# rail-berkeley/serl

Hardware: AMD Instinct MI355X
Metric: learner grad-steps/sec (DrQ, bs256, 2x128x128 img) (higher is better)
Workload: dtype f32 (trunk convs as split-fp16 MFMA x3, fp32 accumulate; <=1e-6 vs fp64); 1 GPU; async_drq_sim (DrQ, ResNet-10 frozen trunk, REDQ-10 critic); workload_key=drq, global_batch=256, per_gpu_batch=256, cameras=2, state_dim=24, act_dim=6, replay_capacity=200000, replay_fill=20000, parallelism=dp1, encoder=resnet-pretrained, trunk_passes_per_grad_step=2, trunk_arithmetic=f16x3, schedule=trunk(i+1) overlapped with update(i) on a 2nd stream; gather(i+2) on a 3rd

## Files before the change

serl_amd/csrc/trunk_f16x3_rowslab.h:

```cpp
#pragma once
#include "trunk_f16x3_dma.h"

namespace serl {

__device__ __forceinline__ void rowtile_epilogue(const ConvArgsB& ab, f32x16 (&acc)[2][2], f32x16 (&accx)[2][2], int m0, int n0,
                                                 int n_img, int wave, int li, int lh) {
  const ConvArgs& a = ab.c;
  constexpr int TM = 2, TN = 2, WROWS = 64;
  const int wrow0 = m0 + wave * WROWS;
  float winv[TN];
#pragma unroll
  for (int tn = 0; tn < TN; ++tn) winv[tn] = ab.winv[n0 + tn * 32 + li];
#pragma unroll
  for (int tm = 0; tm < TM; ++tm)
#pragma unroll
    for (int tn = 0; tn < TN; ++tn)
#pragma unroll
      for (int r = 0; r < 16; ++r) acc[tm][tn][r] = (acc[tm][tn][r] + accx[tm][tn][r] * kLoInv) * winv[tn];
#pragma unroll
  for (int tm = 0; tm < TM; ++tm)
#pragma unroll
    for (int r = 0; r < 16; ++r) {
      const int m = wrow0 + tm * 32 + (r & 3) + 8 * (r >> 2) + 4 * lh;
      float* o = a.out + (size_t)m * a.Cout + n0 + li;
#pragma unroll
      for (int tn = 0; tn < TN; ++tn) o[32 * tn] = acc[tm][tn][r];
    }
  const int gsize = a.Cout / kGnGroups;
  double* stp = a.stats + (size_t)n_img * kGnGroups * 2;
#pragma unroll
  for (int tn = 0; tn < TN; ++tn) {
    float s = 0.f, q = 0.f;
#pragma unroll
    for (int tm = 0; tm < TM; ++tm)
#pragma unroll
      for (int r = 0; r < 16; ++r) {
        const float v = acc[tm][tn][r];
        s += v;
        q += v * v;
      }
    stats_flush(s, q, stp, n0 + tn * 32 + li, gsize, true, false);
  }
}

__device__ __forceinline__ void rowtile_epilogue_t(const ConvArgsB& ab, f32x16 (&acc)[2][2], f32x16 (&accx)[2][2], int m0, int n0,
                                                   int n_img, int wave, int lane, int tile_id, uint8_t* lds) {
  const ConvArgs& a = ab.c;
  const FuseArgs& fz = ab.fz;
  constexpr int TM = 2, TN = 2, WROWS = 64;
  const int li = lane & 31, lh = lane >> 5;
  const int wrow0 = m0 + wave * WROWS;
  if (ab.wprio == 2) __builtin_amdgcn_s_setprio(1);
  float winv[TN];
#pragma unroll
  for (int tn = 0; tn < TN; ++tn) winv[tn] = ab.winv[n0 + tn * 32 + li];
#pragma unroll
  for (int tm = 0; tm < TM; ++tm)
#pragma unroll
    for (int tn = 0; tn < TN; ++tn)
#pragma unroll
      for (int r = 0; r < 16; ++r) acc[tm][tn][r] = (acc[tm][tn][r] + accx[tm][tn][r] * kLoInv) * winv[tn];
  const bool local = fz.expected == 0;
  const int gsize = a.Cout / kGnGroups;
  __shared__ float s_part[4][8];
  __shared__ float s_mr[4][2];
#pragma unroll
  for (int tn = 0; tn < TN; ++tn) {
    float s = 0.f, q = 0.f;
#pragma unroll
    for (int tm = 0; tm < TM; ++tm)
#pragma unroll
      for (int r = 0; r < 16; ++r) { const float v = acc[tm][tn][r]; s += v; q += v * v; }
#pragma unroll
    for (int off = 1; off < 16; off <<= 1) { s += __shfl_xor(s, off); q += __shfl_xor(q, off); }
    s += __shfl_xor(s, 32);
    q += __shfl_xor(q, 32);
    if ((lane & 15) == 0 && lane < 32) {
      s_part[wave][(tn * 2 + (lane >> 4)) * 2] = s;
      s_part[wave][(tn * 2 + (lane >> 4)) * 2 + 1] = q;
    }
  }
  __syncthreads();
  if (!local) gnx_publish<0>(fz, tile_id, wave, lane, &s_part[0][0]);
  float* tile = reinterpret_cast<float*>(lds) + wave * (64 * 64);
#pragma unroll
  for (int tm = 0; tm < TM; ++tm)
#pragma unroll
    for (int tn = 0; tn < TN; ++tn)
#pragma unroll
      for (int r = 0; r < 16; ++r) tile[(tm * 32 + (r & 3) + 8 * (r >> 2) + 4 * lh) * 64 + tn * 32 + li] = acc[tm][tn][r];
  const int g8 = lane & 7, rsub = lane >> 3, c0 = n0 + 8 * g8;
  const size_t rowb = (size_t)a.Cout * 4;
  const uint8_t* res_base = fz.mode == 2 ? fz.res_split + (size_t)wrow0 * rowb + c0 * 4
                                         : reinterpret_cast<const uint8_t*>(fz.res_raw) + (size_t)wrow0 * rowb + c0 * 4;
  u32x4 rres[8][2];
  if (fz.mode >= 2) {
#pragma unroll
    for (int p = 0; p < 8; ++p) {
      const uint8_t* q = res_base + (size_t)(8 * p + rsub) * rowb;
      rres[p][0] = *reinterpret_cast<const u32x4*>(q);
      rres[p][1] = *reinterpret_cast<const u32x4*>(q + 16);
    }
  }
  float sc[8], sh[8], rs[8], rh[8];
  {
    float rstd, mf;
    if (local) {
      const int nseg = gsize >> 4, seg0 = (8 * g8 / gsize) * nseg;
      double s0 = 0.0, s1 = 0.0;
      for (int j = 0; j < nseg; ++j) {
        const int k = 2 * (seg0 + j);
        s0 += (((double)s_part[0][k] + (double)s_part[1][k]) + (double)s_part[2][k]) + (double)s_part[3][k];
        s1 += (((double)s_part[0][k + 1] + (double)s_part[1][k + 1]) + (double)s_part[2][k + 1]) + (double)s_part[3][k + 1];
      }
      const double mean = s0 * fz.gn.inv_count, m2 = s1 * fz.gn.inv_count;
      const float var = fmaxf((float)(m2 - mean * mean), 0.f);
      rstd = rsqrtf(var + 1e-5f); mf = (float)mean;
    } else {
      gnx_collect<0>(fz, tile_id, a.tiles_n, n0, wave, lane, &s_part[0][0], s_mr);
      mf = s_mr[g8 >> 1][0]; rstd = s_mr[g8 >> 1][1];
    }
#pragma unroll
    for (int j = 0; j < 8; ++j) { sc[j] = fz.gn.gamma[c0 + j] * rstd; sh[j] = fz.gn.beta[c0 + j] - mf * sc[j]; rs[j] = 0.f; rh[j] = 0.f; }
    if (fz.mode >= 3) {
#pragma unroll
      for (int j = 0; j < 8; ++j) gn_coef1(fz.res_gn, n_img, c0 + j, rs[j], rh[j]);
    }
  }
  uint8_t* out_base = fz.out_split + (size_t)wrow0 * rowb + c0 * 4;
#pragma unroll
  for (int p = 0; p < 8; ++p) {
    const int row = 8 * p + rsub;
    const float4 t0 = *reinterpret_cast<const float4*>(tile + row * 64 + 8 * g8);
    const float4 t1 = *reinterpret_cast<const float4*>(tile + row * 64 + 8 * g8 + 4);
    float v[8] = {t0.x, t0.y, t0.z, t0.w, t1.x, t1.y, t1.z, t1.w};
#pragma unroll
    for (int j = 0; j < 8; ++j) v[j] = v[j] * sc[j] + sh[j];
    if (fz.mode == 2) {
#pragma unroll
      for (int j = 0; j < 4; ++j) {
        const uint32_t wh = rres[p][0][j], wl = rres[p][1][j];
        const h16x2 hh = __builtin_bit_cast(h16x2, wh), ll = __builtin_bit_cast(h16x2, wl);
        v[2 * j] = ((float)hh[0] + (float)ll[0] * kLoInv) + v[2 * j];
        v[2 * j + 1] = ((float)hh[1] + (float)ll[1] * kLoInv) + v[2 * j + 1];
      }
    } else if (fz.mode >= 3) {
#pragma unroll
      for (int j = 0; j < 8; ++j) {
        const uint32_t wx = rres[p][j >> 2][j & 3];
        const float x = __builtin_bit_cast(float, wx);
        const float y = x * rs[j] + rh[j];
        v[j] = (fz.mode == 4 ? fmaxf(y, 0.f) : y) + v[j];
      }
    }
    u32x4 hi, lo;
#pragma unroll
    for (int j = 0; j < 4; ++j) {
      const float a0 = fmaxf(v[2 * j], 0.f), a1 = fmaxf(v[2 * j + 1], 0.f);
      const h16x2 hp = __builtin_amdgcn_cvt_pkrtz(a0, a1);
      const f32x2 rem = {(a0 - (float)hp[0]) * kLoScale, (a1 - (float)hp[1]) * kLoScale};
      const f16x2 lp = __builtin_convertvector(rem, f16x2);
      hi[j] = __builtin_bit_cast(uint32_t, hp);
      lo[j] = __builtin_bit_cast(uint32_t, lp);
    }
    uint8_t* o = out_base + (size_t)row * rowb;
    *reinterpret_cast<u32x4*>(o) = hi;
    *reinterpret_cast<u32x4*>(o + 16) = lo;
  }
}

constexpr int kRowslabPix = 340;
constexpr int kRowslabLds = 2 * 4 * (kRowslabPix * 16 + 32) + 2 * 3 * 2 * 2 * (64 * 16 + 64);
__global__ __launch_bounds__(256, 2) void conv3x3_rowslab_f16x3_kernel(ConvArgsB ab) {
  const ConvArgs& a = ab.c;
  constexpr int TM = 2, TN = 2, WROWS = 64, BM = 256, BN = 64;
  constexpr int A_REGION = kRowslabPix * 16 + 32, A_BYTES = 4 * A_REGION;
  constexpr int B_HALF = BN * 16 + 64, B_PLANE = 2 * B_HALF, B_TAP = 2 * B_PLANE, B_BYTES = 3 * B_TAP;
  static_assert(2 * A_BYTES + 2 * B_BYTES == kRowslabLds, "LDS size of the launch");
  static_assert(3 * 4096 <= B_BYTES, "three DMA pieces per weight buffer");
  constexpr int AJ = 2;
  static_assert(3 * AJ * 256 >= kRowslabPix * 4, "a slab is fetched in three parts");
  extern __shared__ __attribute__((aligned(16))) uint8_t smemb[];
  uint8_t* const smA = smemb;
  uint8_t* const smB = smemb + 2 * A_BYTES;
  const int tid = threadIdx.x, lane = tid & 63, wave = tid >> 6;
  if (ab.wprio) __builtin_amdgcn_s_setprio(3);
  if (ab.stagger > 0 && blockIdx.x >= 256u && blockIdx.x < 512u)
    for (int i = 0; i < ab.stagger; ++i) __builtin_amdgcn_s_sleep(127);
  const int id = (ab.fz.mode && ab.fz.expected) ? fused_tile(ab.fz, gridDim.x) : xcd_remap((int)blockIdx.x, gridDim.x);
  const int bn = id % a.tiles_n, bm = id / a.tiles_n;
  const int m0 = bm * BM, n0 = bn * BN;
  const int n_img = m0 / a.P, oy0 = (m0 - n_img * a.P) / a.Wo;
  const int pw = a.Wo + 2, npix = (BM / a.Wo + 2) * pw;
  const int c16n = a.Cin >> 4, nchunks = 3 * c16n;
  int rbase[3][AJ];
  unsigned okbits = 0;
  __shared__ float s_gn[2][128];
  if (tid < a.Cin) gn_coef1(a.in_gn, n_img, tid, s_gn[0][tid], s_gn[1][tid]);
#pragma unroll
  for (int part = 0; part < 3; ++part) {
    const int v = part * 256 + tid, pix = v >> 1, kh = v & 1;
    const int sy = pix / pw, sx = pix - sy * pw;
    const int iy = oy0 - 1 + sy, ix = sx - 1;
    const int iyc = min(max(iy, 0), a.Hi - 1), ixc = min(max(ix, 0), a.Wi - 1);
    rbase[part][0] = ((n_img * a.Hi + iyc) * a.Wi + ixc) * a.Cin + 8 * kh;
    rbase[part][1] = rbase[part][0] + 4;
    if (pix < npix && iy == iyc && ix == ixc) okbits |= 3u << (part * AJ);
  }
  __syncthreads();
  u32x4 ra[AJ];

#define SERL_RS_LOAD_A(RA, PART, CG)                                                               \
  _Pragma("unroll") for (int j = 0; j < AJ; ++j)                                                   \
    RA[j] = *reinterpret_cast<const u32x4*>(a.in + rbase[PART][j] + ((CG) << 4));
#define SERL_RS_DMA_B(BG, BKY, BBUF)                                                               \
  _Pragma("unroll") for (int kx = 0; kx < 3; ++kx)                                                 \
    __builtin_amdgcn_global_load_lds((gbl_void_t*)(wdsrc + ((size_t)(((BKY) * 3 + kx) * c16n + (BG)) << 12)), \
                                     (lds_void_t*)(smB + (BBUF) * B_BYTES + kx * 4096 + (tid >> 6) * 1024), 16, 0, 0);
#define SERL_RS_STORE_A(RA, PART, ABUF, CGN)                                                       \
  {                                                                                                \
    const int v_ = (PART) * 256 + tid, kh_ = v_ & 1, cb_ = ((CGN) << 4) + 8 * kh_;                 \
    u32x4 hi_ = {0u, 0u, 0u, 0u}, lo_ = {0u, 0u, 0u, 0u};                                          \
    if ((okbits >> ((PART) * AJ)) & 1u) {                                                          \
      _Pragma("unroll") for (int j = 0; j < 2; ++j) {                                              \
        const float4 x_ = __builtin_bit_cast(float4, RA[j]);                                       \
        const float4 sc_ = *reinterpret_cast<const float4*>(&s_gn[0][cb_ + 4 * j]);                \
        const float4 sh_ = *reinterpret_cast<const float4*>(&s_gn[1][cb_ + 4 * j]);                \
        const float4 y_ = make_float4(fmaxf(x_.x * sc_.x + sh_.x, 0.f), fmaxf(x_.y * sc_.y + sh_.y, 0.f), \
                                      fmaxf(x_.z * sc_.z + sh_.z, 0.f), fmaxf(x_.w * sc_.w + sh_.w, 0.f)); \
        uint2 h2_, l2_;                                                                            \
        split4(y_, h2_, l2_);                                                                      \
        hi_[2 * j] = h2_.x; hi_[2 * j + 1] = h2_.y; lo_[2 * j] = l2_.x; lo_[2 * j + 1] = l2_.y;    \
      }                                                                                            \
    }                                                                                              \
    if (v_ < kRowslabPix * 2) {                                                                    \
      uint8_t* d_ = smA + (ABUF) * A_BYTES + (2 * kh_) * A_REGION + (v_ >> 1) * 16;                \
      *reinterpret_cast<u32x4*>(d_) = hi_;                                                         \
      *reinterpret_cast<u32x4*>(d_ + A_REGION) = lo_;                                              \
    }                                                                                              \
  }
#define SERL_RS_LOADS(CG, KY, RA)                                                                  \
  {                                                                                                \
    const int ncg_ = (KY) == 2 ? (CG) + 1 : (CG), nky_ = (KY) == 2 ? 0 : (KY) + 1;                 \
    const int ncgc_ = min(ncg_, c16n - 1), sn_ = min((CG) + 1, c16n - 1);                          \
    SERL_RS_DMA_B(ncgc_, nky_, ((CG) * 3 + (KY) + 1) & 1)                                          \
    if ((KY) == 0) { SERL_RS_LOAD_A(RA, 0, sn_); } else if ((KY) == 1) { SERL_RS_LOAD_A(RA, 1, sn_); } else { SERL_RS_LOAD_A(RA, 2, sn_); } \
  }
#define SERL_RS_STORES(CG, KY, RA)                                                                 \
  {                                                                                                \
    const int sn2_ = min((CG) + 1, c16n - 1);                                                      \
    if ((KY) == 0) { SERL_RS_STORE_A(RA, 0, ((CG) + 1) & 1, sn2_); } else if ((KY) == 1) { SERL_RS_STORE_A(RA, 1, ((CG) + 1) & 1, sn2_); } \
    else { SERL_RS_STORE_A(RA, 2, ((CG) + 1) & 1, sn2_); }                                         \
  }
#define SERL_RS_COMPUTE(C, CG, KY)                                                                 \
  {                                                                                                \
    const uint8_t* sa = smA + ((CG) & 1) * A_BYTES + (KY) * pw * 16;                               \
    const uint8_t* sb = smB + ((C) & 1) * B_BYTES;                                                 \
    _Pragma("unroll") for (int kx = 0; kx < 3; ++kx) {                                             \
      f16x8 ahi[TM], alo[TM], bhi[TN], blo[TN];                                                    \
      _Pragma("unroll") for (int tm = 0; tm < TM; ++tm) {                                          \
        ahi[tm] = *reinterpret_cast<const f16x8*>(sa + arow[tm] + kx * 16);                        \
        alo[tm] = *reinterpret_cast<const f16x8*>(sa + A_REGION + arow[tm] + kx * 16);             \
      }                                                                                            \
      _Pragma("unroll") for (int tn = 0; tn < TN; ++tn) {                                          \
        bhi[tn] = *reinterpret_cast<const f16x8*>(sb + kx * 4096 + wd_bhi[tn]);                    \
        blo[tn] = *reinterpret_cast<const f16x8*>(sb + kx * 4096 + wd_blo[tn]);                    \
      }                                                                                            \
      _Pragma("unroll") for (int tm = 0; tm < TM; ++tm)                                            \
        _Pragma("unroll") for (int tn = 0; tn < TN; ++tn) {                                        \
          accx[tm][tn] = __builtin_amdgcn_mfma_f32_32x32x16_f16(alo[tm], bhi[tn], accx[tm][tn], 0, 0, 0); \
          accx[tm][tn] = __builtin_amdgcn_mfma_f32_32x32x16_f16(ahi[tm], blo[tn], accx[tm][tn], 0, 0, 0); \
          acc[tm][tn] = __builtin_amdgcn_mfma_f32_32x32x16_f16(ahi[tm], bhi[tn], acc[tm][tn], 0, 0, 0); \
        }                                                                                          \
    }                                                                                              \
  }

  f32x16 acc[TM][TN], accx[TM][TN];
#pragma unroll
  for (int tm = 0; tm < TM; ++tm)
#pragma unroll
    for (int tn = 0; tn < TN; ++tn)
#pragma unroll
      for (int r = 0; r < 16; ++r) { acc[tm][tn][r] = 0.f; accx[tm][tn][r] = 0.f; }

  const int li = lane & 31, lh = lane >> 5;
  int arow[TM];
#pragma unroll
  for (int tm = 0; tm < TM; ++tm) {
    const int r = wave * WROWS + tm * 32 + li;
    const int y = r / a.Wo, x = r - y * a.Wo;
    arow[tm] = 2 * lh * A_REGION + (y * pw + x) * 16;
  }
  int wd_bhi[TN], wd_blo[TN];
#pragma unroll
  for (int tn = 0; tn < TN; ++tn) {
    const int row = tn * 32 + li, sw = (row >> 2) & 3;
    wd_bhi[tn] = row * 64 + ((lh ^ sw) << 4);
    wd_blo[tn] = row * 64 + (((2 + lh) ^ sw) << 4);
  }
  const uint8_t* wdsrc = reinterpret_cast<const uint8_t*>(ab.wdma) + (size_t)(n0 >> 6) * (9 * c16n) * 4096 + (tid >> 6) * 1024 + lane * 16;
  SERL_RS_DMA_B(0, 0, 0)
#pragma unroll
  for (int part = 0; part < 3; ++part) {
    SERL_RS_LOAD_A(ra, part, 0);
    SERL_RS_STORE_A(ra, part, 0, 0);
  }
  __syncthreads();
  int cg = 0, ky = 0;
  for (int c = 0; c < nchunks; ++c) {
    SERL_RS_LOADS(cg, ky, ra);
    SERL_RS_COMPUTE(c, cg, ky);
    SERL_RS_STORES(cg, ky, ra);
    __syncthreads();
    if (++ky == 3) { ky = 0; ++cg; }
  }
#undef SERL_RS_LOAD_A
#undef SERL_RS_DMA_B
#undef SERL_RS_STORE_A
#undef SERL_RS_LOADS
#undef SERL_RS_STORES
#undef SERL_RS_COMPUTE
  rowtile_epilogue_t(ab, acc, accx, m0, n0, n_img, wave, lane, id, smemb);
}

constexpr int kSdPieces = 23;
constexpr int kSdSlab = kSdPieces * 1024, kSdW = 3 * 4096;
constexpr int kSlabDmaLds = 2 * kSdSlab + 2 * kSdW;

template <bool EPT = false>
__global__ __launch_bounds__(256, 2) void conv3x3_slabdma_f16x3_kernel(ConvArgsB ab, const uint8_t* zero_page) {
  const ConvArgs& a = ab.c;
  constexpr int TM = 2, TN = 2, WROWS = 64, BM = 256, BN = 64;
  extern __shared__ __attribute__((aligned(16))) uint8_t smemb[];
  uint8_t* const smS = smemb;
  uint8_t* const smW = smemb + 2 * kSdSlab;
  const int tid = threadIdx.x, lane = tid & 63, wave = __builtin_amdgcn_readfirstlane(tid >> 6);
  if (ab.wprio) __builtin_amdgcn_s_setprio(3);
  if (ab.stagger > 0 && blockIdx.x >= 256u && blockIdx.x < 512u)
    for (int i = 0; i < ab.stagger; ++i) __builtin_amdgcn_s_sleep(127);
  const int id = (ab.fz.mode && ab.fz.expected) ? fused_tile(ab.fz, gridDim.x) : xcd_remap((int)blockIdx.x, gridDim.x);
  const int bn = id % a.tiles_n, bm = id / a.tiles_n;
  const int m0 = bm * BM, n0 = bn * BN;
  const int n_img = m0 / a.P, oy0 = (m0 - n_img * a.P) / a.Wo;
  const int pw = a.Wo == 32 ? 34 : 20;
  const int srows = BM / a.Wo + 2;
  const int c16n = a.Cin >> 4, nchunks = 3 * c16n, nslots = 9 * c16n;
  const uint8_t* in_bytes = reinterpret_cast<const uint8_t*>(a.in);
  const uint8_t* zp = zero_page + (lane & 3) * 16;
  unsigned sbase[6], sok = 0;
#pragma unroll
  for (int j = 0; j < 6; ++j) {
    const int pp = 16 * (wave + 4 * j) + (lane >> 2);
    const int sy = pp / pw, sx = pp - sy * pw;
    const int iy = oy0 - 1 + sy, ix = sx - 1;
    const bool ok = sy < srows && sx < a.Wo + 2 && (unsigned)iy < (unsigned)a.Hi && (unsigned)ix < (unsigned)a.Wi;
    const int u = (lane & 3) ^ ((sx >> 2) & 3);
    sbase[j] = ok ? (unsigned)((((long)(n_img * a.Hi + iy) * a.Wi + ix) * a.Cin) * 4 + u * 16) : 0u;
    sok |= (ok ? 1u : 0u) << j;
  }
  const uint8_t* wsrc = reinterpret_cast<const uint8_t*>(ab.wdma) + (size_t)(n0 >> 6) * nslots * 4096 + wave * 1024 + lane * 16;
#define SERL_SD_SLAB(J, CG, SB)                                                                                       \
  if (wave + 4 * (J) < kSdPieces) {                                                                                   \
    const uint8_t* src_ = ((sok >> (J)) & 1u) ? in_bytes + (size_t)sbase[J] + ((CG) << 6) : zp;                       \
    __builtin_amdgcn_global_load_lds((gbl_void_t*)src_, (lds_void_t*)(smS + (SB) * kSdSlab + (wave + 4 * (J)) * 1024), 16, 0, 0); \
  }
#define SERL_SD_W1(CG, KY, WB, KX)                                                                                    \
    __builtin_amdgcn_global_load_lds((gbl_void_t*)(wsrc + ((size_t)(((KY) * 3 + (KX)) * c16n + (CG)) << 12)),        \
                                     (lds_void_t*)(smW + (WB) * kSdW + (KX) * 4096 + wave * 1024), 16, 0, 0);
#define SERL_SD_W(CG, KY, WB) { SERL_SD_W1(CG, KY, WB, 0) SERL_SD_W1(CG, KY, WB, 1) SERL_SD_W1(CG, KY, WB, 2) }
  f32x16 acc[TM][TN], accx[TM][TN];
#pragma unroll
  for (int tm = 0; tm < TM; ++tm)
#pragma unroll
    for (int tn = 0; tn < TN; ++tn)
#pragma unroll
      for (int r = 0; r < 16; ++r) { acc[tm][tn][r] = 0.f; accx[tm][tn][r] = 0.f; }
  const int li = lane & 31, lh = lane >> 5;
  int ahi[TM][3], alo[TM][3];
#pragma unroll
  for (int tm = 0; tm < TM; ++tm) {
    const int r = wave * WROWS + tm * 32 + li;
    const int y = r / a.Wo, x = r - y * a.Wo;
#pragma unroll
    for (int kx = 0; kx < 3; ++kx) {
      const int f = ((x + kx) >> 2) & 3, pa = y * pw + x + kx;
      ahi[tm][kx] = pa * 64 + (((2 * lh) ^ f) << 4);
      alo[tm][kx] = pa * 64 + (((2 * lh + 1) ^ f) << 4);
    }
  }
  int bhi[TN], blo[TN];
#pragma unroll
  for (int tn = 0; tn < TN; ++tn) {
    const int row = tn * 32 + li, sw = (row >> 2) & 3;
    bhi[tn] = row * 64 + ((lh ^ sw) << 4);
    blo[tn] = row * 64 + (((2 + lh) ^ sw) << 4);
  }
#pragma unroll
  for (int j = 0; j < 6; ++j) SERL_SD_SLAB(j, 0, 0)
  SERL_SD_W(0, 0, 0)
  asm volatile("s_waitcnt vmcnt(0)" ::: "memory");
  asm volatile("s_barrier" ::: "memory");
  int cg = 0, ky = 0;
  for (int c = 0; c < nchunks; ++c) {
    const int ncg = ky == 2 ? cg + 1 : cg, nky = ky == 2 ? 0 : ky + 1;
    const int ncgc = min(ncg, c16n - 1), sn = min(cg + 1, c16n - 1);
    SERL_SD_W(ncgc, nky, (c + 1) & 1)
    if (ky == 0) { SERL_SD_SLAB(0, sn, (cg + 1) & 1) SERL_SD_SLAB(1, sn, (cg + 1) & 1) }
    else if (ky == 1) { SERL_SD_SLAB(2, sn, (cg + 1) & 1) SERL_SD_SLAB(3, sn, (cg + 1) & 1) }
    else { SERL_SD_SLAB(4, sn, (cg + 1) & 1) SERL_SD_SLAB(5, sn, (cg + 1) & 1) }
    const uint8_t* sa = smS + (cg & 1) * kSdSlab + ky * pw * 64;
    const uint8_t* sb = smW + (c & 1) * kSdW;
#pragma unroll
    for (int kx = 0; kx < 3; ++kx) {
      f16x8 fah[TM], fal[TM], fbh[TN], fbl[TN];
#pragma unroll
      for (int tm = 0; tm < TM; ++tm) {
        fah[tm] = *reinterpret_cast<const f16x8*>(sa + ahi[tm][kx]);
        fal[tm] = *reinterpret_cast<const f16x8*>(sa + alo[tm][kx]);
      }
#pragma unroll
      for (int tn = 0; tn < TN; ++tn) {
        fbh[tn] = *reinterpret_cast<const f16x8*>(sb + kx * 4096 + bhi[tn]);
        fbl[tn] = *reinterpret_cast<const f16x8*>(sb + kx * 4096 + blo[tn]);
      }
#pragma unroll
      for (int tm = 0; tm < TM; ++tm)
#pragma unroll
        for (int tn = 0; tn < TN; ++tn) {
          accx[tm][tn] = __builtin_amdgcn_mfma_f32_32x32x16_f16(fal[tm], fbh[tn], accx[tm][tn], 0, 0, 0);
          accx[tm][tn] = __builtin_amdgcn_mfma_f32_32x32x16_f16(fah[tm], fbl[tn], accx[tm][tn], 0, 0, 0);
          acc[tm][tn] = __builtin_amdgcn_mfma_f32_32x32x16_f16(fah[tm], fbh[tn], acc[tm][tn], 0, 0, 0);
        }
    }
    asm volatile("s_waitcnt vmcnt(0) lgkmcnt(0)" ::: "memory");
    asm volatile("s_barrier" ::: "memory");
    __builtin_amdgcn_sched_barrier(0);
    if (++ky == 3) { ky = 0; ++cg; }
  }
#undef SERL_SD_SLAB
#undef SERL_SD_W
  if (EPT) rowtile_epilogue_t(ab, acc, accx, m0, n0, n_img, wave, lane, id, smemb);
  else rowtile_epilogue(ab, acc, accx, m0, n0, n_img, wave, li, lh);
}

}
```

Before: 442.6 grad-steps/s.

## Pipeline slab-DMA conv over a six-tap weight ring with counted vmcnt waits

```diff
diff --git a/serl_amd/csrc/trunk_f16x3_rowslab.h b/serl_amd/csrc/trunk_f16x3_rowslab.h
--- a/serl_amd/csrc/trunk_f16x3_rowslab.h
+++ b/serl_amd/csrc/trunk_f16x3_rowslab.h
@@ -324,16 +324,23 @@
 }
 
 constexpr int kSdPieces = 23;
-constexpr int kSdSlab = kSdPieces * 1024, kSdW = 3 * 4096;
-constexpr int kSlabDmaLds = 2 * kSdSlab + 2 * kSdW;
+constexpr int kSdRingTaps = 6, kSdLead = kSdRingTaps - 1;
+constexpr int kSdSlab = kSdPieces * 1024, kSdRing = kSdRingTaps * 4096;
+constexpr int kSlabDmaLds = 2 * kSdSlab + kSdRing;
+constexpr int sd_vmcnt(int kk) {
+  int n = 0;
+  for (int i = 1; i < kSdLead; ++i) n += 1 + ((kk - i + 9) % 9 < 6 ? 1 : 0);
+  return kk == 0 ? n - 1 : n;
+}
+static_assert(sd_vmcnt(0) == 4 && sd_vmcnt(1) == 5 && sd_vmcnt(4) == 8 && sd_vmcnt(8) == 6, "counted waits of the tap ring");
 
 template <bool EPT = false>
-__global__ __launch_bounds__(256, 2) void conv3x3_slabdma_f16x3_kernel(ConvArgsB ab, const uint8_t* zero_page) {
+__global__ __launch_bounds__(256, 2) __attribute__((amdgpu_num_vgpr(108))) void conv3x3_slabdma_f16x3_kernel(ConvArgsB ab, const uint8_t* zero_page) {
   const ConvArgs& a = ab.c;
   constexpr int TM = 2, TN = 2, WROWS = 64, BM = 256, BN = 64;
   extern __shared__ __attribute__((aligned(16))) uint8_t smemb[];
-  uint8_t* const smS = smemb;
-  uint8_t* const smW = smemb + 2 * kSdSlab;
+  uint8_t* const smW = smemb;
+  uint8_t* const smS = smemb + kSdRing;
   const int tid = threadIdx.x, lane = tid & 63, wave = __builtin_amdgcn_readfirstlane(tid >> 6);
   if (ab.wprio) __builtin_amdgcn_s_setprio(3);
   if (ab.stagger > 0 && blockIdx.x >= 256u && blockIdx.x < 512u)
@@ -344,13 +351,14 @@
   const int n_img = m0 / a.P, oy0 = (m0 - n_img * a.P) / a.Wo;
   const int pw = a.Wo == 32 ? 34 : 20;
   const int srows = BM / a.Wo + 2;
-  const int c16n = a.Cin >> 4, nchunks = 3 * c16n, nslots = 9 * c16n;
+  const int c16n = a.Cin >> 4, nslots = 9 * c16n;
   const uint8_t* in_bytes = reinterpret_cast<const uint8_t*>(a.in);
   const uint8_t* zp = zero_page + (lane & 3) * 16;
   unsigned sbase[6], sok = 0;
 #pragma unroll
   for (int j = 0; j < 6; ++j) {
-    const int pp = 16 * (wave + 4 * j) + (lane >> 2);
+    const int pc = wave + 4 * j < kSdPieces ? wave + 4 * j : wave + 4 * j - 4;
+    const int pp = 16 * pc + (lane >> 2);
     const int sy = pp / pw, sx = pp - sy * pw;
     const int iy = oy0 - 1 + sy, ix = sx - 1;
     const bool ok = sy < srows && sx < a.Wo + 2 && (unsigned)iy < (unsigned)a.Hi && (unsigned)ix < (unsigned)a.Wi;
@@ -360,14 +368,16 @@
   }
   const uint8_t* wsrc = reinterpret_cast<const uint8_t*>(ab.wdma) + (size_t)(n0 >> 6) * nslots * 4096 + wave * 1024 + lane * 16;
 #define SERL_SD_SLAB(J, CG, SB)                                                                                       \
-  if (wave + 4 * (J) < kSdPieces) {                                                                                   \
-    const uint8_t* src_ = ((sok >> (J)) & 1u) ? in_bytes + (size_t)sbase[J] + ((CG) << 6) : zp;                       \
-    __builtin_amdgcn_global_load_lds((gbl_void_t*)src_, (lds_void_t*)(smS + (SB) * kSdSlab + (wave + 4 * (J)) * 1024), 16, 0, 0); \
-  }
-#define SERL_SD_W1(CG, KY, WB, KX)                                                                                    \
-    __builtin_amdgcn_global_load_lds((gbl_void_t*)(wsrc + ((size_t)(((KY) * 3 + (KX)) * c16n + (CG)) << 12)),        \
-                                     (lds_void_t*)(smW + (WB) * kSdW + (KX) * 4096 + wave * 1024), 16, 0, 0);
-#define SERL_SD_W(CG, KY, WB) { SERL_SD_W1(CG, KY, WB, 0) SERL_SD_W1(CG, KY, WB, 1) SERL_SD_W1(CG, KY, WB, 2) }
+  {                                                                                                                   \
+    const int pc_ = wave + 4 * (J) < kSdPieces ? wave + 4 * (J) : wave + 4 * (J) - 4;                                 \
+     \
+    unsigned so_ = sbase[J];                                                                                          \
+    asm volatile("" : "+v"(so_));                                                                                     \
+    const uint8_t* src_ = ((sok >> (J)) & 1u) ? in_bytes + (size_t)so_ + ((CG) << 6) : zp;                            \
+    __builtin_amdgcn_global_load_lds((gbl_void_t*)src_, (lds_void_t*)(smS + (SB) * kSdSlab + pc_ * 1024), 16, 0, 0);  \
+  }
+#define SERL_SD_W(SLOT, POS)                                                                                          \
+    __builtin_amdgcn_global_load_lds((gbl_void_t*)(wsrc + ((size_t)(SLOT) << 12)), (lds_void_t*)(smW + (POS) * 4096 + wave * 1024), 16, 0, 0);
   f32x16 acc[TM][TN], accx[TM][TN];
 #pragma unroll
   for (int tm = 0; tm < TM; ++tm)
@@ -376,18 +386,18 @@
 #pragma unroll
       for (int r = 0; r < 16; ++r) { acc[tm][tn][r] = 0.f; accx[tm][tn][r] = 0.f; }
   const int li = lane & 31, lh = lane >> 5;
-  int ahi[TM][3], alo[TM][3];
-#pragma unroll
-  for (int tm = 0; tm < TM; ++tm) {
-    const int r = wave * WROWS + tm * 32 + li;
+  int ahi[3], alo[3];
+  {
+    const int r = wave * WROWS + li;
     const int y = r / a.Wo, x = r - y * a.Wo;
 #pragma unroll
     for (int kx = 0; kx < 3; ++kx) {
       const int f = ((x + kx) >> 2) & 3, pa = y * pw + x + kx;
-      ahi[tm][kx] = pa * 64 + (((2 * lh) ^ f) << 4);
-      alo[tm][kx] = pa * 64 + (((2 * lh + 1) ^ f) << 4);
-    }
-  }
+      ahi[kx] = pa * 64 + (((2 * lh) ^ f) << 4);
+      alo[kx] = pa * 64 + (((2 * lh + 1) ^ f) << 4);
+    }
+  }
+  const int tmo = (32 / a.Wo) * pw * 64;
   int bhi[TN], blo[TN];
 #pragma unroll
   for (int tn = 0; tn < TN; ++tn) {
@@ -395,48 +405,76 @@
     bhi[tn] = row * 64 + ((lh ^ sw) << 4);
     blo[tn] = row * 64 + (((2 + lh) ^ sw) << 4);
   }
+#define SERL_SD_READ_A(SET, KA)                                                                                       \
+  {                                                                                                                   \
+    constexpr int ga_ = (KA) / 9, kya_ = ((KA) % 9) / 3, kxa_ = (KA) % 3;                                             \
+                              \
+    _Pragma("unroll") for (int tm = 0; tm < TM; ++tm) {                                                               \
+      int kyo_ = kya_ * pw * 64 + tm * tmo;                                                                           \
+      asm volatile("" : "+s"(kyo_));                                                                                  \
+      const uint8_t* sa = smS + ga_ * kSdSlab + kyo_;                                                                 \
+      fa[SET][2 * tm] = *reinterpret_cast<const f16x8*>(sa + ahi[kxa_]);                                              \
+      fa[SET][2 * tm + 1] = *reinterpret_cast<const f16x8*>(sa + alo[kxa_]);                                          \
+    }                                                                                                                 \
+  }
+#define SERL_SD_MFMA(TM_, TN_)                                                                                        \
+    accx[TM_][TN_] = __builtin_amdgcn_mfma_f32_32x32x16_f16(fa[cur_][2 * (TM_) + 1], fbh[TN_], accx[TM_][TN_], 0, 0, 0); \
+    acc[TM_][TN_] = __builtin_amdgcn_mfma_f32_32x32x16_f16(fa[cur_][2 * (TM_)], fbh[TN_], acc[TM_][TN_], 0, 0, 0);    \
+    accx[TM_][TN_] = __builtin_amdgcn_mfma_f32_32x32x16_f16(fa[cur_][2 * (TM_)], fbl[TN_], accx[TM_][TN_], 0, 0, 0);
+#define SERL_SD_TAP(K)                                                                                                \
+  {                                                                                                                   \
+    constexpr int g_ = (K) / 9, kk_ = (K) % 9, u_ = (K) + kSdLead, cur_ = (K) & 1;                                    \
+    const uint8_t* sb = smW + ((K) % kSdRingTaps) * 4096;                                                             \
+     \
+    __builtin_amdgcn_sched_barrier(0);                                                                                \
+    asm volatile("s_waitcnt vmcnt(%0) lgkmcnt(0)" ::"n"(sd_vmcnt(kk_)) : "memory");                                   \
+    asm volatile("s_barrier" ::: "memory");                                                                           \
+    __builtin_amdgcn_sched_barrier(0);                                                                                \
+    f16x8 fbh[TN], fbl[TN];                                                                                           \
+    _Pragma("unroll") for (int tn = 0; tn < TN; ++tn) {                                                               \
+      fbh[tn] = *reinterpret_cast<const f16x8*>(sb + bhi[tn]);                                                        \
+      fbl[tn] = *reinterpret_cast<const f16x8*>(sb + blo[tn]);                                                        \
+    }                                                                                                                 \
+    if (kk_ == 0) SERL_SD_READ_A(cur_, K)       \
+                                                \
+    __builtin_amdgcn_sched_barrier(0);                                                                                \
+    if (kk_ < 6) SERL_SD_SLAB((kk_ < 6 ? kk_ : 0), min(cg0 + g_ + 1, c16n - 1), (g_ + 1) & 1)                         \
+    {                                                                                                                 \
+      const int wcg_ = cg0 + u_ / 9;                                                                                  \
+      const int slot_ = wcg_ < c16n ? (u_ % 9) * c16n + wcg_ : nslots - 1;                                            \
+      SERL_SD_W(slot_, u_ % kSdRingTaps)                                                                              \
+    }                                                                                                                 \
+    __builtin_amdgcn_sched_barrier(0);                                                                                \
+    SERL_SD_MFMA(0, 0)                                                                                                \
+     \
+    __builtin_amdgcn_sched_barrier(0);                                                                                \
+    if (kk_ != 8) SERL_SD_READ_A(1 - cur_, (K) + 1)                                                                   \
+    __builtin_amdgcn_sched_barrier(0);                                                                                \
+    SERL_SD_MFMA(0, 1) SERL_SD_MFMA(1, 0) SERL_SD_MFMA(1, 1)                                                          \
+                 \
+    asm volatile("" ::"v"(acc[0][0]), "v"(acc[0][1]), "v"(acc[1][0]), "v"(acc[1][1]), "v"(accx[0][0]), "v"(accx[0][1]), \
+                 "v"(accx[1][0]), "v"(accx[1][1]));                                                                   \
+  }
+  f16x8 fa[2][2 * TM];
 #pragma unroll
   for (int j = 0; j < 6; ++j) SERL_SD_SLAB(j, 0, 0)
-  SERL_SD_W(0, 0, 0)
-  asm volatile("s_waitcnt vmcnt(0)" ::: "memory");
+#pragma unroll
+  for (int t = 0; t < kSdLead; ++t) SERL_SD_W(t * c16n, t)
+  int cg0 = 0;
+  for (; cg0 + 1 < c16n; cg0 += 2) {
+    SERL_SD_TAP(0) SERL_SD_TAP(1) SERL_SD_TAP(2) SERL_SD_TAP(3) SERL_SD_TAP(4) SERL_SD_TAP(5) SERL_SD_TAP(6) SERL_SD_TAP(7) SERL_SD_TAP(8)
+    SERL_SD_TAP(9) SERL_SD_TAP(10) SERL_SD_TAP(11) SERL_SD_TAP(12) SERL_SD_TAP(13) SERL_SD_TAP(14) SERL_SD_TAP(15) SERL_SD_TAP(16) SERL_SD_TAP(17)
+  }
+  if (cg0 < c16n) {
+    SERL_SD_TAP(0) SERL_SD_TAP(1) SERL_SD_TAP(2) SERL_SD_TAP(3) SERL_SD_TAP(4) SERL_SD_TAP(5) SERL_SD_TAP(6) SERL_SD_TAP(7) SERL_SD_TAP(8)
+  }
+  __builtin_amdgcn_sched_barrier(0);
+  asm volatile("s_waitcnt vmcnt(0) lgkmcnt(0)" ::: "memory");
   asm volatile("s_barrier" ::: "memory");
-  int cg = 0, ky = 0;
-  for (int c = 0; c < nchunks; ++c) {
-    const int ncg = ky == 2 ? cg + 1 : cg, nky = ky == 2 ? 0 : ky + 1;
-    const int ncgc = min(ncg, c16n - 1), sn = min(cg + 1, c16n - 1);
-    SERL_SD_W(ncgc, nky, (c + 1) & 1)
-    if (ky == 0) { SERL_SD_SLAB(0, sn, (cg + 1) & 1) SERL_SD_SLAB(1, sn, (cg + 1) & 1) }
-    else if (ky == 1) { SERL_SD_SLAB(2, sn, (cg + 1) & 1) SERL_SD_SLAB(3, sn, (cg + 1) & 1) }
-    else { SERL_SD_SLAB(4, sn, (cg + 1) & 1) SERL_SD_SLAB(5, sn, (cg + 1) & 1) }
-    const uint8_t* sa = smS + (cg & 1) * kSdSlab + ky * pw * 64;
-    const uint8_t* sb = smW + (c & 1) * kSdW;
-#pragma unroll
-    for (int kx = 0; kx < 3; ++kx) {
-      f16x8 fah[TM], fal[TM], fbh[TN], fbl[TN];
-#pragma unroll
-      for (int tm = 0; tm < TM; ++tm) {
-        fah[tm] = *reinterpret_cast<const f16x8*>(sa + ahi[tm][kx]);
-        fal[tm] = *reinterpret_cast<const f16x8*>(sa + alo[tm][kx]);
-      }
-#pragma unroll
-      for (int tn = 0; tn < TN; ++tn) {
-        fbh[tn] = *reinterpret_cast<const f16x8*>(sb + kx * 4096 + bhi[tn]);
-        fbl[tn] = *reinterpret_cast<const f16x8*>(sb + kx * 4096 + blo[tn]);
-      }
-#pragma unroll
-      for (int tm = 0; tm < TM; ++tm)
-#pragma unroll
-        for (int tn = 0; tn < TN; ++tn) {
-          accx[tm][tn] = __builtin_amdgcn_mfma_f32_32x32x16_f16(fal[tm], fbh[tn], accx[tm][tn], 0, 0, 0);
-          accx[tm][tn] = __builtin_amdgcn_mfma_f32_32x32x16_f16(fah[tm], fbl[tn], accx[tm][tn], 0, 0, 0);
-          acc[tm][tn] = __builtin_amdgcn_mfma_f32_32x32x16_f16(fah[tm], fbh[tn], acc[tm][tn], 0, 0, 0);
-        }
-    }
-    asm volatile("s_waitcnt vmcnt(0) lgkmcnt(0)" ::: "memory");
-    asm volatile("s_barrier" ::: "memory");
-    __builtin_amdgcn_sched_barrier(0);
-    if (++ky == 3) { ky = 0; ++cg; }
-  }
+  __builtin_amdgcn_sched_barrier(0);
+#undef SERL_SD_TAP
+#undef SERL_SD_MFMA
+#undef SERL_SD_READ_A
 #undef SERL_SD_SLAB
 #undef SERL_SD_W
   if (EPT) rowtile_epilogue_t(ab, acc, accx, m0, n0, n_img, wave, lane, id, smemb);
```

After: 446.7 grad-steps/s, median of 6. No clear change (+0.9%).
